# DUBSON0/iterative-closest-point-avmi

Hardware: AMD Instinct MI355X
Metric: icp_iterations_per_sec (higher is better)
Workload: dtype f64

## Files before the change

iterative-closest-point-avmi_amd/csrc/icp2.hip:

```cpp
#include <cstdlib>

#include "linalg.hpp"
#include "prep_common.hpp"
#include "sweep.hpp"

namespace icpmi {


struct Icp2Args {
    const double* pts;
    const int32_t* off;
    const int32_t* cnt;
    const int32_t* pair_src;
    const int32_t* pair_tgt;
    const double* init;
    double* results;
    const double2* g_sxy;
    const double2* g_snrm;
    const int32_t* g_sorig;
    const float* g_skey;
    const int32_t* g_dir;
    int lds_points;
    double error_threshold;
    double max_corr_dist;
    int max_iterations;
    int method;
    int has_init;
    int n_lo, m_lo;
    int skip_over;
    int it_begin, it_limit;
    int resume;
    double2* st_xy;
    int32_t* st_pos;
    int32_t* list;
    int32_t* list_count;
    int st_stride;
    int32_t* wide_list;
    int32_t* wide_count;
    int32_t* far_list;
    int32_t* far_count;
    double far_d2;
    IcpGate gate;
};
constexpr int ICP2_FAR_THREADS = 1024, ICP2_FAR_SMAX = 2, ICP2_FAR_POINTS = 2048;
constexpr int ICP2_ST_PARKED = 100;

__device__ __forceinline__ double swap_add(double a, double b, bool rows16) {
    const long long ab = __double_as_longlong(a), bb = __double_as_longlong(b);
    const unsigned alo = (unsigned)ab, ahi = (unsigned)(ab >> 32), blo = (unsigned)bb, bhi = (unsigned)(bb >> 32);
    unsigned xl, xh, yl, yh;
    if (rows16) {
        const auto r0 = __builtin_amdgcn_permlane16_swap(alo, blo, false, false);
        const auto r1 = __builtin_amdgcn_permlane16_swap(ahi, bhi, false, false);
        xl = r0[0]; yl = r0[1]; xh = r1[0]; yh = r1[1];
    } else {
        const auto r0 = __builtin_amdgcn_permlane32_swap(alo, blo, false, false);
        const auto r1 = __builtin_amdgcn_permlane32_swap(ahi, bhi, false, false);
        xl = r0[0]; yl = r0[1]; xh = r1[0]; yh = r1[1];
    }
    return __longlong_as_double(((long long)xh << 32) | xl) + __longlong_as_double(((long long)yh << 32) | yl);
}

constexpr int RED_MAXW = 16;
template <int NV>
constexpr int red_doubles() { return (NV + 3) / 4 * 4 * RED_MAXW; }

template <int NV>
__device__ __forceinline__ void wave_totals(double* scratch, const double (&v)[NV]) {
    constexpr int NP = (NV + 3) / 4 * 4;
    const int w = wave_id(), l = lane_id();
    double h[NP / 2];
#pragma unroll
    for (int j = 0; j < NP / 2; ++j)
        h[j] = swap_add(2 * j < NV ? v[2 * j] : 0.0, 2 * j + 1 < NV ? v[2 * j + 1] : 0.0, false);
#pragma unroll
    for (int k = 0; k < NP / 4; ++k) {
        const double q = row_sum(swap_add(h[2 * k], h[2 * k + 1], true));
        const int row = l >> 4;
        const int idx = 4 * k + ((row & 1) << 1) + (row >> 1);
        if ((l & 15) == 0 && idx < NV) scratch[idx * RED_MAXW + w] = q;
    }
}

template <int NV>
// ... 68 lines not shown
    ctrl[CTRL_TT] = (tt0 * r[0] + tt1 * r[1]) + t[0]; ctrl[CTRL_TT + 1] = (tt0 * r[2] + tt1 * r[3]) + t[1];
}

union FarSlot {
    struct { double x, y; int seed, pad; } in;
    struct { double s1, s3; int p1, p2; } out;
};
static_assert(sizeof(FarSlot) == 24, "24 B per row");

template <int THREADS, int ICP2_SMAX, bool TGT_LDS, bool FILT, bool RESUME, bool FAR = false>
__device__ __forceinline__ void icp2_pair(const Icp2Args& a, const int b) {
    extern __shared__ __attribute__((aligned(16))) unsigned char dyn[];
    __shared__ double redA[red_doubles<11>()];
    __shared__ double redB[red_doubles<4>()];
    __shared__ double ctrl[CTRL_DOUBLES];
    constexpr int NWAVES = THREADS / ICPMI_WAVE;

    const int tid = threadIdx.x;
    const bool lead = tid < ICPMI_WAVE;
    const int sc = a.pair_src[b], tc = a.pair_tgt[b];
    const int N = a.cnt ? a.cnt[sc] : a.off[sc + 1] - a.off[sc];
    const int M = a.cnt ? a.cnt[tc] : a.off[tc + 1] - a.off[tc];
    const double* src = a.pts + (size_t)a.off[sc] * 2;
    double* res = a.results + (size_t)b * ICPMI_RES_DOUBLES;
    const int dir = a.g_dir[tc];
    if (a.skip_over ? (N > THREADS * ICP2_SMAX || (TGT_LDS && M > a.lds_points)) : (a.n_lo >= 0 && N <= a.n_lo && M <= a.m_lo)) {
        if (a.skip_over && a.wide_list && threadIdx.x == 0) a.wide_list[atomicAdd(a.wide_count, 1)] = b;
        return;
    }
    const int gate_index = a.gate.base + b * a.gate.stride;
    if (RESUME && a.gate.hint) {
        __shared__ int gate_skip;
        if (tid == 0) {
            gate_skip = __hip_atomic_load(a.gate.hint, __ATOMIC_RELAXED, __HIP_MEMORY_SCOPE_AGENT) < gate_index;
            if (gate_skip) {
                res[ICPMI_RES_ITERS] += 1.0;
                res[ICPMI_RES_STATUS] = (double)ICPMI_ST_SKIPPED;
            }
        }
        __syncthreads();
        if (gate_skip) return;
    }

    double2* lds_xy = reinterpret_cast<double2*>(dyn);
    double2* lds_nrm = reinterpret_cast<double2*>(dyn + (size_t)a.lds_points * 16);
    int32_t* lds_orig = reinterpret_cast<int32_t*>(dyn + (size_t)a.lds_points * 32);
    float4* lds_sq = reinterpret_cast<float4*>(dyn + (size_t)a.lds_points * 32) + 1;
    const double2* sxy = TGT_LDS ? lds_xy : a.g_sxy + a.off[tc];
    const double2* snrm = TGT_LDS ? lds_nrm : a.g_snrm + a.off[tc];
    const int32_t* sorig = TGT_LDS ? lds_orig : a.g_sorig + a.off[tc];
    static_assert(TGT_LDS || !FILT, "the filter images live in LDS");
    static_assert(!FAR || (FILT && RESUME), "the far continuation: filter images, parked state");
    float4* lds_tree = reinterpret_cast<float4*>(dyn + (size_t)a.lds_points * 48 + 32);
    const int tree_leaves = sweepf_tree_leaves(M);
    FarSlot* far_q = reinterpret_cast<FarSlot*>(dyn + (size_t)a.lds_points * 50 + 32) + (size_t)(threadIdx.x / ICPMI_WAVE) * (ICPMI_WAVE * ICP2_SMAX);
    __shared__ int rt_bits;
    if (FILT && tid == 0) rt_bits = 0;

    if (tid == 0) {
        if (RESUME) {
            ctrl[CTRL_RT] = res[0]; ctrl[CTRL_RT + 1] = res[1]; ctrl[CTRL_RT + 2] = res[2]; ctrl[CTRL_RT + 3] = res[3];
            ctrl[CTRL_TT] = res[ICPMI_RES_T]; ctrl[CTRL_TT + 1] = res[ICPMI_RES_T + 1];
            ctrl[CTRL_ERR] = res[ICPMI_RES_ERR]; ctrl[CTRL_PREV] = res[ICPMI_RES_ERR]; ctrl[CTRL_DELTA] = res[ICPMI_RES_DELTA];
            ctrl[CTRL_ITERS] = res[ICPMI_RES_ITERS];
        } else {
            const double* in = a.init + (size_t)b * 6;
            ctrl[CTRL_RT] = a.has_init ? in[0] : 1.0; ctrl[CTRL_RT + 1] = a.has_init ? in[1] : 0.0;
            ctrl[CTRL_RT + 2] = a.has_init ? in[2] : 0.0; ctrl[CTRL_RT + 3] = a.has_init ? in[3] : 1.0;
            ctrl[CTRL_TT] = a.has_init ? in[4] : 0.0; ctrl[CTRL_TT + 1] = a.has_init ? in[5] : 0.0;
            ctrl[CTRL_ERR] = __builtin_inf(); ctrl[CTRL_PREV] = __builtin_inf(); ctrl[CTRL_DELTA] = __builtin_inf();
            ctrl[CTRL_ITERS] = 0.0;
        }
        ctrl[CTRL_STATUS] = (double)ICPMI_ST_MAXITER;
    }

    if (N <= 0 || M <= 0 || dir < 0 || (TGT_LDS && M > a.lds_points) || N > THREADS * ICP2_SMAX || (!FILT && dir >= SWEEP_POLAR)) {
        if (tid == 0) ctrl[CTRL_STATUS] = (double)ICPMI_ST_EMPTY;
    } else {
        const bool use_p2l = a.method == ICPMI_POINT_TO_LINE;
        const double2* gx = a.g_sxy + a.off[tc];
        const double2* gn = a.g_snrm + a.off[tc];
        const int32_t* go = a.g_sorig + a.off[tc];
        const float* gk = a.g_skey + a.off[tc];
        SweepF filt{0.0, 0.0, 0.0, 0.0f, 0.0f};
        if constexpr (TGT_LDS && !FILT)
            for (int i = tid; i < M; i += THREADS) {
                lds_xy[i] = gx[i];
                lds_orig[i] = go[i];
                if (use_p2l) lds_nrm[i] = gn[i];
            }
        if constexpr (FILT) {
            if (dir != SWEEP_POLAR) {
                const double2 o = gx[M >> 1];
                filt.ox = wave_uniform(o.x); filt.oy = wave_uniform(o.y); filt.uo = wave_uniform(proj(dir, o.x, o.y));
            }
            float rmax = 0.0f;
            for (int i = tid; i < M; i += THREADS) {
                const double2 p = gx[i];
                lds_xy[i] = p;
                if (use_p2l) lds_nrm[i] = gn[i];
                const float4 q = make_float4((float)(p.x - filt.ox), (float)(p.y - filt.oy),
                                             dir == SWEEP_POLAR ? gk[i] : (float)(proj(dir, p.x, p.y) - filt.uo),
                                             __int_as_float(go[i]));
                lds_sq[i] = q;
                rmax = fmaxf(rmax, fmaxf(fabsf(q.x), fabsf(q.y)));
            }
            if (tid == 0) { lds_sq[-1] = make_float4(0.f, 0.f, 0.f, 0.f); lds_sq[M] = make_float4(0.f, 0.f, 0.f, 0.f); }
            __syncthreads();
            atomicMax(&rt_bits, __float_as_int(rmax));
        }
        double px[ICP2_SMAX], py[ICP2_SMAX];
        int pos[ICP2_SMAX];
        float ax[ICP2_SMAX], ay[ICP2_SMAX], budget[ICP2_SMAX];
        int pos2[ICP2_SMAX];
#pragma unroll
        for (int s = 0; s < ICP2_SMAX; ++s) { ax[s] = 0.0f; ay[s] = 0.0f; budget[s] = -1.0f; pos2[s] = -1; }
        const int S = (N + THREADS - 1) / THREADS;
#pragma unroll
        for (int s = 0; s < ICP2_SMAX; ++s) {
            const int n = s * THREADS + tid;
            px[s] = 0.0; py[s] = 0.0; pos[s] = -1;
            if (n < N && RESUME) {
                const double2 v = a.st_xy[(size_t)b * a.st_stride + n];
                px[s] = v.x; py[s] = v.y; pos[s] = a.st_pos[(size_t)b * a.st_stride + n];
            } else if (n < N) {
                const double x = src[2 * n], y = src[2 * n + 1];
                if (a.has_init) {
                    const double* in = a.init + (size_t)b * 6;
                    double sx = 0.0, sy = 0.0;
                    sx += x * in[0]; sx += y * in[1]; sx += in[4];
                    sy += x * in[2]; sy += y * in[3]; sy += in[5];
                    px[s] = sx; py[s] = sy;
                } else { px[s] = x; py[s] = y; }
            }
        }
        const bool has_corr = a.max_corr_dist >= 0.0;
        const double max_corr_sq = wave_uniform(a.max_corr_dist * a.max_corr_dist);
        const int need = max(3, N / 10);
        __syncthreads();
        if constexpr (FAR) {
            sweepf_build_tree(lds_sq, M, lds_tree, tree_leaves, tid, THREADS);
            __syncthreads();
        }
        const double2 c_lo = sxy[0], c_hi = sxy[M - 1];
        const double uabs = wave_uniform(fmax(fabs(proj(dir, c_lo.x, c_lo.y)), fabs(proj(dir, c_hi.x, c_hi.y))));
        if constexpr (FILT) {
            filt.rt = wave_uniform(__int_as_float(rt_bits) * 1.000001f);
            filt.ut = wave_uniform(fmaxf(fabsf(lds_sq[0].z), fabsf(lds_sq[M - 1].z)) * 1.000001f);
        }

        double e_part = 0.0;
        if (RESUME) {
#pragma unroll
            for (int s = 0; s < ICP2_SMAX; ++s) {
                if (!(s < S && s * THREADS + tid < N)) continue;
                const double2 q = sxy[pos[s]];
                const double ex = q.x - px[s], ey = q.y - py[s];
                double se = 0.0;
                se += ex * ex;
                se += ey * ey;
                e_part += se;
            }
// ... 58 lines not shown
                                pos[s] = sweepf_nn_pk(lds_sq, sxy, filt, M, dir, uabs, px[s], py[s], pos[s], it < ICP2_PLAIN_CENTRED);
                            else pos[s] = sweepf_nn(lds_sq, sxy, filt, M, dir, uabs, px[s], py[s], pos[s], it < ICP2_PLAIN_CENTRED, d2s);
                        }
                        else pos[s] = sweep_nn(sxy, sorig, M, dir, uabs, px[s], py[s], pos[s], it < ICP2_PLAIN_CENTRED, d2s);
                    }
            } else {
                const bool centred = !RESUME && it < ICP2_CENTRED_ITERS;
                int slot[ICP2_SMAX];
                if constexpr (FAR) {
                    int nq = 0;
#pragma unroll
                    for (int s = 0; s < ICP2_SMAX; ++s) {
                        const unsigned long long bal = __ballot(srch[s]);
                        slot[s] = nq + (int)__builtin_amdgcn_mbcnt_hi((unsigned)(bal >> 32), __builtin_amdgcn_mbcnt_lo((unsigned)bal, 0u));
                        nq += __popcll(bal);
                        if (srch[s]) {
                            FarSlot e;
                            e.in.x = px[s]; e.in.y = py[s]; e.in.seed = pos[s]; e.in.pad = 0;
                            far_q[slot[s]] = e;
                        }
                    }
                    __builtin_amdgcn_fence(__ATOMIC_ACQ_REL, "wavefront");
                    __builtin_amdgcn_wave_barrier();
                    for (int j = tid & (ICPMI_WAVE - 1); j < nq; j += ICPMI_WAVE) {
                        const FarSlot e = far_q[j];
                        const Top2 r = sweepf_top2_far(lds_sq, sxy, lds_tree, tree_leaves, filt, M, dir, uabs, e.in.x, e.in.y, e.in.seed);
                        FarSlot o;
                        o.out.s1 = r.s1; o.out.s3 = r.s3; o.out.p1 = r.p1; o.out.p2 = r.p2;
                        far_q[j] = o;
                    }
                    __builtin_amdgcn_fence(__ATOMIC_ACQ_REL, "wavefront");
                    __builtin_amdgcn_wave_barrier();
                }
#pragma unroll
                for (int s = 0; s < ICP2_SMAX; ++s)
                    if (srch[s]) {
                        Top2 t2;
                        if constexpr (FAR) {
                            const FarSlot o = far_q[slot[s]];
                            t2.p1 = o.out.p1; t2.p2 = o.out.p2; t2.s1 = o.out.s1; t2.s2 = o.out.s1; t2.s3 = o.out.s3;
                        }
                        else if constexpr (FILT) {
                            if (__popcll(__ballot(true)) >= ICP2_PK_MIN)
                                t2 = sweepf_top2_pk(lds_sq, sxy, filt, M, dir, uabs, px[s], py[s], pos[s], centred);
                            else t2 = sweepf_top2(lds_sq, sxy, filt, M, dir, uabs, px[s], py[s], pos[s], centred);
                        }
                        else t2 = sweep_top2(sxy, sorig, M, dir, uabs, px[s], py[s], pos[s], centred);
                        pos[s] = t2.p1; pos2[s] = t2.p2;
                        float bf;
                        if constexpr (FAR) {
                            const double d1 = sqrt(t2.s1), d3 = sqrt(t2.s3);
                            bf = (float)(d3 - 1e-13 * (d3 + d1) - 1.3e-7 * (fabs(px[s]) + fabs(py[s])));
                        } else {
                            const float r3 = __builtin_amdgcn_sqrtf((float)t2.s3) * 0.9999997f;
                            const float r1 = __builtin_amdgcn_sqrtf((float)t2.s1) * 1.0000003f + 1e-30f;
                            bf = (r3 - r1) * 0.4999999f - 1.3e-7f * (fabsf((float)px[s]) + fabsf((float)py[s]));
                        }
                        bf = bf - fabsf(bf) * 1e-6f;
                        budget[s] = t2.s3 < __builtin_inf() ? bf : __builtin_inff();
                        ax[s] = (float)px[s]; ay[s] = (float)py[s];
                    }
            }
            bool in[ICP2_SMAX];
#pragma unroll
            for (int s = 0; s < ICP2_SMAX; ++s) in[s] = s < S && s * THREADS + tid < N;
            if (use_p2l) {
                double acc[11] = {0, 0, 0, 0, 0, 0, 0, 0, 0, 0, 0};
#pragma unroll
                for (int s = 0; s < ICP2_SMAX; ++s) {
                    if (!in[s]) continue;
                    const double2 q = sxy[pos[s]], nm = snrm[pos[s]];
                    const double dx = px[s] - q.x, dy = py[s] - q.y;
                    if (has_corr) {
                        double s2 = 0.0;
                        s2 += dx * dx;
                        s2 += dy * dy;
                        const double dist = sqrt(s2);
                        if (!(dist * dist < max_corr_sq)) continue;
                    }
                    const double c = nm.y * px[s] - nm.x * py[s];
                    const double bi = -(nm.x * dx + nm.y * dy);
                    acc[0] += c * c;       acc[1] += c * nm.x;    acc[2] += c * nm.y;
                    acc[3] += nm.x * nm.x; acc[4] += nm.x * nm.y; acc[5] += nm.y * nm.y;
                    acc[6] += c * bi;      acc[7] += nm.x * bi;   acc[8] += nm.y * bi;
                    acc[9] += 1.0;
                }
                acc[10] = e_part;
                wave_totals<11>(redA, acc);
                __syncthreads();
                if (lead) {
                    combine_totals<11>(redA, NWAVES, acc);
                    const int fin = gate_stop(ctrl, a.gate.hint, gate_seen, gate_index, tid == 0,
                                              finish_step(ctrl, it, acc[10], acc[9], N, has_corr, need, a.error_threshold, tid == 0, far_err));
                    const bool stop = fin == FIN_STOP;
                    if (!stop) {
                        double A[3][3] = {{acc[0], acc[1], acc[2]}, {acc[1], acc[3], acc[4]}, {acc[2], acc[4], acc[5]}};
                        double rhs[3] = {acc[6], acc[7], acc[8]}, x[3];
                        double r[4], t[2];
                        if (solve3(A, rhs, x)) {
                            double st, ct;
                            sincos_step(x[0], st, ct);
                            r[0] = ct; r[1] = -st; r[2] = st; r[3] = ct; t[0] = x[1]; t[1] = x[2];
                        } else {
                            r[0] = 1.0; r[1] = 0.0; r[2] = 0.0; r[3] = 1.0; t[0] = 0.0; t[1] = 0.0;
                        }
                        if (tid == 0) {
                            accumulate_step(ctrl, r, t);
                            ctrl[CTRL_R] = r[0]; ctrl[CTRL_R + 1] = r[1]; ctrl[CTRL_R + 2] = r[2]; ctrl[CTRL_R + 3] = r[3];
                            ctrl[CTRL_T] = t[0]; ctrl[CTRL_T + 1] = t[1];
// ... 156 lines not shown
    for (int j = first + blockIdx.x; j < count; j += gridDim.x) {
        icp2_pair<THREADS, ICP2_SMAX, TGT_LDS, FILT, true>(a, __builtin_amdgcn_readfirstlane(a.list[j]));
        __syncthreads();
    }
}

__global__ __launch_bounds__(ICP2_FAR_THREADS, 4) void icp2_far_kernel(Icp2Args a) {
    const int count = *a.far_count;
    for (int j = blockIdx.x; j < count; j += gridDim.x) {
        icp2_pair<ICP2_FAR_THREADS, ICP2_FAR_SMAX, true, true, true, true>(a, __builtin_amdgcn_readfirstlane(a.far_list[j]));
        __syncthreads();
    }
}

struct Icp2Ws {
    Carve c;
    int n_pairs, max_src_n;
    size_t st_rows = (size_t)n_pairs * (size_t)max_src_n;
    double2* st_xy = c.packed<double2>(st_rows * 16);
    int32_t* st_pos = c.packed<int32_t>(st_rows * 4);
    int32_t *list = c.packed<int32_t>((size_t)n_pairs * 4), *wide_list = c.packed<int32_t>((size_t)n_pairs * 4);
    int32_t* far_list = c.packed<int32_t>((size_t)n_pairs * 4);
    int32_t* list_count = c.packed<int32_t>(64);
    size_t bytes = c.off;
};


struct Icp2Shape {
    int threads, smax;
    bool in_lds, filter;
    int lds_points;
    size_t lds;
    int n_lo, m_lo;
    int skip_over;
};
struct Icp2Plan {
    Icp2Shape first;
    bool has_wide;
    Icp2Shape wide;
    bool two_stage;
    int stage1_iterations, stage2_grid, wide_grid;
    bool far_wanted;
    Icp2Shape far;
    double far_d2;
    bool needs_lists;
};
constexpr int ICP2_NO_LIMIT = 0x7fffffff;

static Icp2Shape icp2_shape(int threads, int smax, int points, bool in_lds) {
    int cap = 64;
    while (cap < points) cap <<= 1;
    if (points > 1024 && points <= 1536) cap = 1536;
    const bool filter = in_lds && cap <= 2048;
    const size_t lds = in_lds ? (filter ? (size_t)cap * 48 + 32 : (size_t)cap * 36) : 0;
    return {threads, smax, in_lds, filter, cap, lds, -1, 0, 0};
}

static Icp2Plan plan_icp2(int n_pairs, int max_src_n, int max_tgt_n, const icpmi_icp_params& p, bool have_ws,
                          const char* stages_opt, const char* far_opt) {
    Icp2Plan plan{};
    const bool in_lds = max_tgt_n <= 4096;
    const bool many = n_pairs >= 1024;
    int T, SM;
    if (max_src_n <= 1024) { T = 512; SM = 2; }
    else if (many) { T = 768; SM = 2; }
    else if (max_src_n <= 2048) { T = 1024; SM = 2; }
    else { T = 1024; SM = 4; }
    const int cap1 = ((T == 512 || T == 768) && many && in_lds && max_tgt_n > 1536) ? 1536 : max_tgt_n;
    plan.first = icp2_shape(T, SM, cap1, in_lds);
    plan.has_wide = T * SM < max_src_n || cap1 < max_tgt_n;
    if (plan.has_wide) {
        plan.first.skip_over = 1;
        plan.wide = icp2_shape(1024, max_src_n <= 2048 ? 2 : 4, max_tgt_n, in_lds);
        plan.wide.n_lo = T * SM; plan.wide.m_lo = cap1;
    }
    plan.stage1_iterations = ICP2_STAGE1_ITERS;
    plan.two_stage = many && have_ws && p.max_iterations >= 2 * plan.stage1_iterations &&
                     !(stages_opt && stages_opt[0] == '1') &&
                     (p.method == ICPMI_POINT_TO_LINE || (stages_opt && stages_opt[0] == '2'));
    plan.stage2_grid = n_pairs / 8 > 256 ? n_pairs / 8 : 256;
    plan.wide_grid = n_pairs < 256 ? n_pairs : (n_pairs / 32 > 256 ? n_pairs / 32 : 256);
    plan.far_d2 = far_opt ? atof(far_opt) : 1.0;
    plan.far_wanted = have_ws && in_lds && plan.far_d2 > 0.0 && p.max_iterations > 2;
    int far_cap = 64;
    while (far_cap < max_tgt_n && far_cap < ICP2_FAR_POINTS) far_cap <<= 1;
    plan.far = {ICP2_FAR_THREADS, ICP2_FAR_SMAX, true, true, far_cap,
                (size_t)far_cap * 50 + 32 + sizeof(FarSlot) * (size_t)(ICP2_FAR_THREADS * ICP2_FAR_SMAX), -1, 0, 0};
    plan.needs_lists = have_ws && (plan.two_stage || plan.has_wide);
    return plan;
}

struct Icp2Kernels {
    void (*fused)(Icp2Args);
    void (*wide)(Icp2Args);
    void (*resume)(Icp2Args);
    void (*resume_rest)(Icp2Args, int);
};
template <int T, int S, bool L, bool F>
constexpr Icp2Kernels icp2_kernels() {
    return {icp2_fused_kernel<T, S, L, F>, icp2_wide_kernel<T, S, L, F>, icp2_resume_kernel<T, S, L, F>,
            icp2_resume_rest_kernel<T, S, L, F>};
}
template <int T, int S>
static Icp2Kernels icp2_kernels_of(const Icp2Shape& s) {
    if (!s.in_lds) return icp2_kernels<T, S, false, false>();
    if (s.filter) return icp2_kernels<T, S, true, true>();
    return icp2_kernels<T, S, true, false>();
}
static Icp2Kernels icp2_kernels_of(const Icp2Shape& s) {
    if (s.threads == 512 && s.smax == 2) return icp2_kernels_of<512, 2>(s);
    if (s.threads == 768 && s.smax == 2) return icp2_kernels_of<768, 2>(s);
    if (s.threads == 1024 && s.smax == 2) return icp2_kernels_of<1024, 2>(s);
    if (s.threads == 1024 && s.smax == 4) return icp2_kernels_of<1024, 4>(s);
    return {nullptr, nullptr, nullptr, nullptr};
}

static Icp2Args icp2_args(const Icp2Args& base, const Icp2Shape& s, int it_begin, int it_limit, int resume) {
    Icp2Args a = base;
    a.lds_points = s.lds_points; a.n_lo = s.n_lo; a.m_lo = s.m_lo; a.skip_over = s.skip_over;
    a.it_begin = it_begin; a.it_limit = it_limit; a.resume = resume;
    return a;
}

int launch_icp2(const double* pts, const int32_t* off, const int32_t* cnt, const int32_t* ps, const int32_t* pt,
                int n_pairs, int max_src_n, int max_tgt_n, int total_rows, const icpmi_icp_params* p, const double* init,
                double* results, const void* prepared, void* workspace, size_t workspace_bytes, const IcpGate* gate,
                hipStream_t st) {
    const Icp2Ws w{workspace, n_pairs, max_src_n};
    const bool have_ws = workspace && workspace_bytes >= w.bytes;
    const Icp2Plan plan = plan_icp2(n_pairs, max_src_n, max_tgt_n, *p, have_ws, option("ICP2_STAGES"), option("ICP2_FAR"));
    const Icp2Kernels k1 = icp2_kernels_of(plan.first), k2 = icp2_kernels_of(plan.wide);
    if (!k1.fused || (plan.has_wide && !k2.fused)) return ICPMI_ERR_ARG;
    Icp2Args base;
    base.gate = gate ? *gate : IcpGate{nullptr, nullptr, 0.0, 0, 1};
    base.st_xy = nullptr; base.st_pos = nullptr; base.list = nullptr; base.list_count = nullptr; base.st_stride = 0;
    base.wide_list = nullptr; base.wide_count = nullptr;
    base.far_list = nullptr; base.far_count = nullptr; base.far_d2 = __builtin_inf();
    const PreparedView v(prepared, total_rows);
    base.pts = pts; base.off = off; base.cnt = cnt; base.pair_src = ps; base.pair_tgt = pt; base.init = init; base.results = results;
    base.g_sxy = v.sxy; base.g_snrm = v.snrm; base.g_sorig = v.sorig; base.g_skey = v.skey; base.g_dir = v.dir;
    base.error_threshold = p->error_threshold; base.max_corr_dist = p->max_corr_dist;
    base.max_iterations = p->max_iterations; base.method = p->method; base.has_init = p->has_init;
    const bool far_go = plan.far_wanted && dyn_lds((const void*)icp2_far_kernel, plan.far.lds) == hipSuccess;
    if (plan.needs_lists || far_go) {
        base.st_xy = w.st_xy; base.st_pos = w.st_pos; base.st_stride = max_src_n;
        base.list = w.list; base.list_count = w.list_count;
        if (plan.has_wide) { base.wide_list = w.wide_list; base.wide_count = w.list_count + 1; }
        if (far_go) { base.far_list = w.far_list; base.far_count = w.list_count + 2; base.far_d2 = plan.far_d2; }
        if (hipMemsetAsync(w.list_count, 0, 3 * sizeof(int32_t), st) != hipSuccess) return ICPMI_ERR_HIP;
    }
    SideLock side_lock;
    Side* const side = side_lock.side;

    const Icp2Shape& s1 = plan.first;
    if (dyn_lds((const void*)k1.fused, s1.lds) != hipSuccess) return ICPMI_ERR_HIP;
    k1.fused<<<n_pairs, s1.threads, s1.lds, st>>>(
        icp2_args(base, s1, 0, plan.two_stage ? plan.stage1_iterations : ICP2_NO_LIMIT, 0));
    bool forked = false;
    if (plan.two_stage) {
        if (base.wide_list && side) forked = hipEventRecord(side->fork, st) == hipSuccess;
        const Icp2Args second = icp2_args(base, s1, plan.stage1_iterations, ICP2_NO_LIMIT, 1);
        if (dyn_lds((const void*)k1.resume, s1.lds) != hipSuccess) return ICPMI_ERR_HIP;
        k1.resume<<<plan.stage2_grid, s1.threads, s1.lds, st>>>(second);
        if (plan.stage2_grid < n_pairs) {
            if (dyn_lds((const void*)k1.resume_rest, s1.lds) != hipSuccess) return ICPMI_ERR_HIP;
            k1.resume_rest<<<256, s1.threads, s1.lds, st>>>(second, plan.stage2_grid);
        }
    }
    if (plan.has_wide) {
        const Icp2Shape& s2 = plan.wide;
        const Icp2Args wide = icp2_args(base, s2, 0, ICP2_NO_LIMIT, 0);
        if (base.wide_list) {
            if (dyn_lds((const void*)k2.wide, s2.lds) != hipSuccess) return ICPMI_ERR_HIP;
            hipStream_t ws = st;
            if (forked && hipStreamWaitEvent(side->stream[0], side->fork, 0) == hipSuccess) ws = side->stream[0];
            k2.wide<<<plan.wide_grid, s2.threads, s2.lds, ws>>>(wide);
            if (ws != st && (hipEventRecord(side->join[0], ws) != hipSuccess ||
                             hipStreamWaitEvent(st, side->join[0], 0) != hipSuccess)) {
                (void)hipStreamSynchronize(ws);
                return ICPMI_ERR_HIP;
            }
        } else {
            if (dyn_lds((const void*)k2.fused, s2.lds) != hipSuccess) return ICPMI_ERR_HIP;
            k2.fused<<<n_pairs, s2.threads, s2.lds, st>>>(wide);
        }
    }
    if (base.far_list)
// ... 8 lines not shown
```

iterative-closest-point-avmi_amd/csrc/prep.hip:

```cpp
#include "prep_common.hpp"

namespace icpmi {

#ifndef PREP_AXIS_STEP
#define PREP_AXIS_STEP 4
#endif
#ifndef ICPMI_PREP_WPS
#define ICPMI_PREP_WPS 6
#endif
constexpr int PREP_THREADS = 512;
constexpr int PREP_MAXW = PREP_THREADS / ICPMI_WAVE;
constexpr int PREP_MAX_POINTS = 4096;

constexpr float PREP_POLAR_Q = 6.283185307179586f / 2097152.0f;
__device__ __forceinline__ uint32_t prep_polar_key21(double x, double y) {
    const float t = (atan2f((float)y, (float)x) + 3.14159265f) * (2097152.0f / 6.283185307179586f);
    const int k = (int)t;
    return (uint32_t)(k < 0 ? 0 : (k > 2097151 ? 2097151 : k));
}
__device__ __forceinline__ float prep_polar_image(uint32_t k21) { return (float)k21 * PREP_POLAR_Q - 3.14159265f; }

template <int E>
__device__ __forceinline__ void prep_sort_polar32(const double* __restrict__ P, int M, uint64_t* keys, uint32_t* rows) {
    uint32_t v[E];
#pragma unroll
    for (int e = 0; e < E; ++e) {
        const int i = e * PREP_THREADS + (int)threadIdx.x;
        v[e] = i < M ? (prep_polar_key21(P[2 * i], P[2 * i + 1]) << 11) | (uint32_t)i : 0xffffffffu;
    }
    bitonic_sort_regs_fixed<uint32_t, E, PREP_THREADS>(v, reinterpret_cast<uint32_t*>(keys));
    __syncthreads();
#pragma unroll
    for (int e = 0; e < E; ++e) {
        const int i = (int)threadIdx.x * E + e;
        rows[i] = v[e] == 0xffffffffu ? 0xffffffffu : (v[e] & 0x7ffu);
        keys[i] = v[e] == 0xffffffffu ? ~0ull : f64_sortable((double)prep_polar_image(v[e] >> 11));
    }
    __syncthreads();
}

template <int E>
__device__ __forceinline__ void prep_sort_regs(const double* __restrict__ P, int M, int dir, uint64_t* by_row, uint64_t* keys,
                                               uint32_t* rows) {
    if (dir == SWEEP_POLAR) { prep_sort_polar32<E>(P, M, keys, rows); return; }
    constexpr uint64_t ROW_MASK = 0x7ff;
    uint64_t v[E];
#pragma unroll
    for (int e = 0; e < E; ++e) {
        const int i = (int)threadIdx.x * E + e;
        const uint64_t k = i < M ? f64_sortable(proj(dir, P[2 * i], P[2 * i + 1])) : ~0ull;
        by_row[i] = k;
        v[e] = i < M ? ((k & ~ROW_MASK) | (uint64_t)i) : ~0ull;
    }
    bitonic_sort_regs_fixed<uint64_t, E, PREP_THREADS>(v, keys);
    int bad = 0;
#pragma unroll
    for (int e = 0; e < E; ++e) {
        const int i = (int)threadIdx.x * E + e;
        const uint32_t r = v[e] == ~0ull ? 0xffffffffu : (uint32_t)(v[e] & ROW_MASK);
        rows[i] = r;
        keys[i] = r == 0xffffffffu ? ~0ull : by_row[r];
    }
    __syncthreads();
#pragma unroll
    for (int e = 0; e < E; ++e) {
        const int i = (int)threadIdx.x * E + e;
        if (i + 1 < M && (keys[i] > keys[i + 1] || (keys[i] == keys[i + 1] && rows[i] > rows[i + 1]))) bad = 1;
    }
    if (__syncthreads_or(bad)) {
        if (threadIdx.x == 0)
            for (int i = 1; i < M; ++i) {
                const uint64_t k = keys[i];
                const uint32_t r = rows[i];
                int j = i - 1;
                while (j >= 0 && (keys[j] > k || (keys[j] == k && rows[j] > r))) { keys[j + 1] = keys[j]; rows[j + 1] = rows[j]; --j; }
                keys[j + 1] = k; rows[j + 1] = r;
            }
        __syncthreads();
    }
}

template <int KK, bool GRID>
__global__ __launch_bounds__(PREP_THREADS, (KK <= 13 ? ICPMI_PREP_WPS : (KK <= 16 ? 4 : 2))) void prep_targets_kernel(
    const double* __restrict__ pts, const int32_t* __restrict__ off, const int32_t* __restrict__ cnt,
    const int32_t* __restrict__ cloud_ids, int k, double2* __restrict__ g_sxy, double2* __restrict__ g_snrm,
    int32_t* __restrict__ g_sorig, float* __restrict__ g_skey, int32_t* __restrict__ g_dir, double* __restrict__ out_normals,
    int lds_points, int split, int polar) {
    extern __shared__ __attribute__((aligned(16))) unsigned char dyn[];
    __shared__ double dsc[8 * PREP_MAXW];
// ... 276 lines not shown
```

iterative-closest-point-avmi_amd/csrc/state.hip:

```cpp
#include <link.h>

#include <cstdio>
#include <cstdlib>
#include <cstring>
#include <map>
#include <set>
#include <mutex>
#include <string>

#include "common.hpp"

namespace icpmi {

static const char* const kOptionNames[] = {"ICP2_SIDE", "ICP2_FAR", "ICP2_STAGES", "POLAR", "PREP_KNN", "RAYCAST", "RS_BATCH"};

struct Options {
    std::mutex mu;
    bool loaded = false;
    std::map<std::string, std::string> values;
    void load() {
        if (loaded) return;
        loaded = true;
        for (const char* n : kOptionNames) {
            const std::string env = std::string("ICPMI_") + n;
            if (const char* v = getenv(env.c_str())) values[n] = v;
        }
    }
};
static Options& options() { static Options o; return o; }

static const char* strip_prefix(const char* name) { return strncmp(name, "ICPMI_", 6) == 0 ? name + 6 : name; }

const char* option(const char* name) {
    Options& o = options();
    std::lock_guard<std::mutex> g(o.mu);
    o.load();
    const auto it = o.values.find(strip_prefix(name));
    return it == o.values.end() ? nullptr : it->second.c_str();
}

struct LdsAttr {
    std::mutex mu;
    std::map<std::pair<const void*, int>, size_t> granted;
};
static LdsAttr& lds_attr() { static LdsAttr a; return a; }

hipError_t dyn_lds(const void* fn, size_t bytes) {
    int dev = -1;
    hipError_t e = hipGetDevice(&dev);
    if (e != hipSuccess) return e;
    LdsAttr& a = lds_attr();
    std::lock_guard<std::mutex> g(a.mu);
    size_t& have = a.granted[std::make_pair(fn, dev)];
    if (bytes <= have) return hipSuccess;
    e = hipFuncSetAttribute(fn, hipFuncAttributeMaxDynamicSharedMemorySize, (int)bytes);
    if (e == hipSuccess) have = bytes;
    return e;
}

struct SideState {
    std::mutex mu;
    std::map<int, Side> per_device;
};
static SideState& side_state() { static SideState s; return s; }

SideLock::SideLock() : side(nullptr) {
    SideState& s = side_state();
// ... 74 lines not shown
```

iterative-closest-point-avmi_amd/csrc/sweep.hpp:

```cpp
#pragma once
#include "common.hpp"

namespace icpmi {

__device__ __forceinline__ double proj(int dir, double x, double y) {
    const double a = dir == 1 ? 0.0 : 1.0;
    const double b = dir == 0 ? 0.0 : (dir == 3 ? -1.0 : 1.0);
    return x * a + y * b;
}

__device__ __forceinline__ bool gap_exceeds(int dir, double uq, double uc, double bound_d2) {
    const double du = fabs(uq - uc);
    if (dir < 2) return du * du > bound_d2;
    const double e = 4.5e-16 * (fabs(uq) + fabs(uc));
    const double l = du - e;
    return l > 0.0 && l * l > bound_d2 * 2.000000000000002;
}

__device__ __forceinline__ int sweep_lower_bound(const double2* sxy, int m, int dir, double uq) {
    int lo = 0, hi = m;
    while (lo < hi) {
        const int mid = (lo + hi) >> 1;
        const double2 c = sxy[mid];
        if (proj(dir, c.x, c.y) < uq) lo = mid + 1; else hi = mid;
// ... 136 lines not shown
        lo = inl ? lo - 1 : -1;
        cr = nr; cl = nl;
    }
    return t;
}

__device__ __forceinline__ int sweep_nn(const double2* sxy, const int32_t* sorig, int m, int dir, double uabs,
                                        double qx, double qy, int seed, bool CENTRED, double& d2_out) {
    const SweepAxis ax(dir, qx, qy, uabs);
    double best = __builtin_inf(), thr = __builtin_inf();
    int bpos = 0;
    int lo, hi;
    const bool seeded = seed >= 0 && seed < m;
    if (seeded) {
        best = sweep_d2(qx, qy, sxy[seed]); bpos = seed;
        thr = ax.width(best);
    }
    if (seeded && !CENTRED) { lo = seed - 1; hi = seed + 1; }
    else {
        hi = sweep_lower_bound(sxy, m, dir, ax.uq);
        lo = hi - 1;
    }
    double2 cr = sweep_load(sxy, hi, m), cl = sweep_load(sxy, lo, m);
    while (lo >= 0 || hi < m) {
        const double2 nr = sweep_load(sxy, hi + 1, m), nl = sweep_load(sxy, lo - 1, m);
        const bool inr = hi < m && !(ax.u(cr) - ax.uq > thr);
        const bool inl = lo >= 0 && !(ax.uq - ax.u(cl) > thr);
        const double sr = sweep_d2(qx, qy, cr), sl = sweep_d2(qx, qy, cl);
#pragma unroll
        for (int side = 0; side < 2; ++side) {
            const int i = side == 0 ? hi : lo;
            const double s = side == 0 ? sr : sl;
            const bool take = side == 0 ? inr : inl;
            if (take && s == best && i != bpos) {
                if (sorig[i] < sorig[bpos]) bpos = i;
            }
            const bool lt = take && s < best;
            best = lt ? s : best;
            bpos = lt ? i : bpos;
        }
        thr = ax.width(best);
        hi = inr ? hi + 1 : m;
        lo = inl ? lo - 1 : -1;
        cr = nr; cl = nl;
    }
    d2_out = best;
    return bpos;
}


constexpr int SWEEP_POLAR = 4;
__device__ __forceinline__ double polar_key(double x, double y) { return atan2(y, x); }

struct SweepF {
    double ox, oy, uo;
    float ut, rt;
};
struct SweepFQuery {
    float x, y, u;
    float e15, mu;
    float kw;
    bool polar;
    __device__ __forceinline__ SweepFQuery(const SweepF& f, int dir, double uabs, double qx, double qy) {
        polar = dir == SWEEP_POLAR;
        x = (float)(qx - f.ox); y = (float)(qy - f.oy);
        e15 = 1.8e-7f * (fabsf(x) + fabsf(y) + 2.0f * f.rt) + 1e-30f;
        if (polar) {
            u = atan2f(y, x);
            mu = 1e-5f;
            kw = 1.00001f / __builtin_amdgcn_sqrtf(x * x + y * y);
        } else {
            const SweepAxis ax(dir, qx, qy, uabs);
            u = (float)(ax.uq - f.uo);
            mu = 2.4e-7f * (fabsf(u) + f.ut) + (float)ax.slack * 1.000001f + 1e-30f;
            kw = dir < 2 ? 1.0f : 1.4142137f;
        }
    }
    __device__ __forceinline__ void bounds(double best, float& W, float& T) const {
        const float B = __builtin_amdgcn_sqrtf((float)best) * 1.000001f + 1e-18f;
        const float t = B * kw;
        if (polar) W = t <= 0.7f ? (t + 0.3f * t * t * t) * 1.000001f + mu : __builtin_inff();
        else W = t * 1.000001f + mu;
        const float b = B + e15;
        T = b * b * 1.000002f;
    }
};

typedef float sweep_v2f __attribute__((ext_vector_type(2)));

__device__ __forceinline__ int sweepf_row(const float4 c) { return __float_as_int(c.w); }

__device__ __forceinline__ int sweepf_lower_bound(const float4* sq, int m, float u) {
    int lo = 0, hi = m;
    while (lo < hi) {
        const int mid = (lo + hi) >> 1;
        if (sq[mid].z < u) lo = mid + 1; else hi = mid;
    }
    return lo;
}

struct SweepFWalk {
    int lo, hi, lo_end, hi_end;
    bool openr, openl;
    sweep_v2f uu;
    __device__ __forceinline__ SweepFWalk(int lo0, int hi0, int m, float u) {
        lo = lo0; hi = hi0; lo_end = -1; hi_end = m; openr = true; openl = true;
        uu = sweep_v2f{-u, u};
    }
    __device__ __forceinline__ bool more() const { return (openr && hi < hi_end) || (openl && lo > lo_end); }
    __device__ __forceinline__ bool wrap(int m) {
        const bool endr = openr && hi >= hi_end, endl = openl && lo <= lo_end;
        if (endr == endl) return false;
        if (endr) { hi_end = lo + 1; hi = 0; uu.x += 6.2831855f; openl = false; lo_end = lo; }
        else { lo_end = hi - 1; lo = m - 1; uu.y += 6.2831855f; openr = false; hi_end = hi; }
        return hi < hi_end || lo > lo_end;
    }
};

struct SweepFRound {
    bool inr, inl, pr, pl;
    float4 cr, cl;
    __device__ __forceinline__ SweepFRound(const float4* sq, const SweepFWalk& w, const SweepFQuery& fq, float W, float T) {
        cr = sq[w.hi]; cl = sq[w.lo];
        const sweep_v2f cz = {cr.z, -cl.z};
        const sweep_v2f g = cz + w.uu;
        inr = w.openr && w.hi < w.hi_end && !(g.x > W);
        inl = w.openl && w.lo > w.lo_end && !(g.y > W);
        const sweep_v2f cx = {cr.x, cl.x}, cy = {cr.y, cl.y};
        const sweep_v2f dx = fq.x - cx, dy = fq.y - cy;
        const sweep_v2f s2 = __builtin_elementwise_fma(dx, dx, dy * dy);
        pr = inr && !(s2.x > T);
        pl = inl && !(s2.y > T);
    }
    __device__ __forceinline__ void advance(SweepFWalk& w) const {
        w.openr = w.openr && (inr || w.hi >= w.hi_end);
        w.openl = w.openl && (inl || w.lo <= w.lo_end);
        w.hi += inr ? 1 : 0;
        w.lo -= inl ? 1 : 0;
    }
};

__device__ __forceinline__ int sweepf_nn(const float4* sq, const double2* sxy, const SweepF& f, int m, int dir, double uabs,
                                         double qx, double qy, int seed, bool CENTRED, double& d2_out) {
    const SweepFQuery fq(f, dir, uabs, qx, qy);
    double best = __builtin_inf();
    float W = __builtin_inff(), T = __builtin_inff();
    int bpos = 0;
    const bool seeded = seed >= 0 && seed < m;
    if (seeded) {
        best = sweep_d2(qx, qy, sxy[seed]); bpos = seed;
        fq.bounds(best, W, T);
    }
    const bool from_seed = seeded && !CENTRED && !(fq.polar && fabsf(sq[seed].z - fq.u) > 3.0f);
    const int h0 = from_seed ? seed + 1 : sweepf_lower_bound(sq, m, fq.u);
    SweepFWalk w(from_seed ? seed - 1 : h0 - 1, h0, m, fq.u);
#pragma unroll 1
    for (int pass = 0; pass < 2; ++pass) {
        while (w.more()) {
            const SweepFRound r(sq, w, fq, W, T);
            if (r.pr || r.pl) {
#pragma unroll
                for (int side = 0; side < 2; ++side) {
                    const int i = side == 0 ? w.hi : w.lo;
                    if (side == 0 ? r.pr : r.pl) {
                        const double s = sweep_d2(qx, qy, sxy[i]);
                        if (s == best && i != bpos) {
                            if (sweepf_row(side == 0 ? r.cr : r.cl) < sweepf_row(sq[bpos])) bpos = i;
                        }
                        if (s < best) { best = s; bpos = i; }
                    }
                }
                fq.bounds(best, W, T);
            }
            r.advance(w);
        }
        if (!fq.polar || !w.wrap(m)) break;
    }
    d2_out = best;
    return bpos;
}

__device__ __forceinline__ Top2 sweepf_top2(const float4* sq, const double2* sxy, const SweepF& f, int m, int dir, double uabs,
                                            double qx, double qy, int seed, bool CENTRED) {
    const SweepFQuery fq(f, dir, uabs, qx, qy);
    Top2 t;
    t.p1 = 0; t.p2 = -1;
    t.s1 = t.s2 = t.s3 = __builtin_inf();
    float W = __builtin_inff(), T = __builtin_inff();
    const bool seeded = seed >= 0 && seed < m;
    if (seeded) { t.s1 = sweep_d2(qx, qy, sxy[seed]); t.p1 = seed; }
    const bool from_seed = seeded && !CENTRED && !(fq.polar && fabsf(sq[seed].z - fq.u) > 3.0f);
    const int h0 = from_seed ? seed + 1 : sweepf_lower_bound(sq, m, fq.u);
    SweepFWalk w(from_seed ? seed - 1 : h0 - 1, h0, m, fq.u);
    const int skip = seeded ? seed : -1;
#pragma unroll 1
    for (int pass = 0; pass < 2; ++pass) {
        while (w.more()) {
            const SweepFRound r(sq, w, fq, W, T);
            const bool pr = r.pr && w.hi != skip, pl = r.pl && w.lo != skip;
            if (pr || pl) {
#pragma unroll
                for (int side = 0; side < 2; ++side) {
                    const int i = side == 0 ? w.hi : w.lo;
                    if (side == 0 ? pr : pl) {
                        const double s = sweep_d2(qx, qy, sxy[i]);
                        if (s == t.s1 || s == t.s2) {
                            const int row = sweepf_row(side == 0 ? r.cr : r.cl), r1 = sweepf_row(sq[t.p1]);
                            const int r2 = t.p2 >= 0 ? sweepf_row(sq[t.p2]) : 0x7fffffff;
                            if (s < t.s1 || (s == t.s1 && row < r1)) { t.s3 = t.s2; t.s2 = t.s1; t.p2 = t.p1; t.s1 = s; t.p1 = i; }
                            else if (s < t.s2 || row < r2) { t.s3 = t.s2; t.s2 = s; t.p2 = i; }
                            else t.s3 = s;
                        } else {
                            const bool c1 = s < t.s1, c2 = s < t.s2, c3 = s < t.s3;
                            t.s3 = c2 ? t.s2 : (c3 ? s : t.s3);
                            t.s2 = c1 ? t.s1 : (c2 ? s : t.s2);
                            t.p2 = c1 ? t.p1 : (c2 ? i : t.p2);
                            t.s1 = c1 ? s : t.s1;
                            t.p1 = c1 ? i : t.p1;
                        }
                    }
                }
                fq.bounds(t.s3, W, T);
            }
            r.advance(w);
        }
        if (!fq.polar || !w.wrap(m)) break;
    }
    return t;
}

constexpr unsigned SWEEP_PK_IDX = 0x7FFu;
constexpr unsigned SWEEP_PK_NONE = 0xFFFFFFFFu;

__device__ __forceinline__ unsigned sweep_med3_u32(unsigned a, unsigned b, unsigned c) {
    unsigned r;
    asm("v_med3_u32 %0, %1, %2, %3" : "=v"(r) : "v"(a), "v"(b), "v"(c));
    return r;
}
__device__ __forceinline__ unsigned sweep_min_u32(unsigned a, unsigned b) { return a < b ? a : b; }

template <int K>
struct SweepPkList {
    unsigned m[K];
    __device__ __forceinline__ SweepPkList() {
#pragma unroll
// ... 24 lines not shown
    __device__ __forceinline__ float width(float B) const {
        const float t = B * kw;
        if (POLAR) {
            const float w = __builtin_fmaf(t, __builtin_fmaf(0.3000004f, t * t, 1.000001f), mu);
            return t <= 0.7f ? w : __builtin_inff();
        }
        return __builtin_fmaf(t, 1.000001f, mu);
    }
    __device__ __forceinline__ float threshold(float B) const {
        const float b = B + e15;
        return b * b * 1.000002f;
    }
};

template <int K, int NB, bool POLAR>
__device__ __forceinline__ bool sweep_pk_walk(const float4* sq, const SweepPkQuery& fq, int lo, int hi, int m, int skip, SweepPkList<K>& L,
                                              int max_rounds = 0) {
    float W = fq.width<POLAR>(fq.dist_bound(L.m[NB]));
    const float ur = -fq.u, ul = fq.u, ur2 = 6.2831855f - fq.u, ul2 = fq.u + 6.2831855f;
    int rounds = 0;
    for (;;) {
        int hp = hi, lp = lo;
        float o_r = ur, o_l = ul;
        bool okr, okl;
        if (POLAR) {
            const bool wr = hi >= m, wl = lo < 0;
            hp = wr ? hi - m : hi;
            lp = wl ? lo + m : lo;
            o_r = wr ? ur2 : ur;
            o_l = wl ? ul2 : ul;
            okr = hi - lo <= m;
        } else {
            okr = hi < m;
            okl = lo >= 0;
        }
        const float4 cr = sq[hp], cl = sq[lp];
        const bool inr = okr && !(cr.z + o_r > W);
        if (POLAR) okl = hi + (inr ? 1 : 0) - lo <= m;
        const bool inl = okl && !(o_l - cl.z > W);
        const sweep_v2f cx = {cr.x, cl.x}, cy = {cr.y, cl.y};
        const sweep_v2f dx = fq.x - cx, dy = fq.y - cy;
        const sweep_v2f s2 = __builtin_elementwise_fma(dx, dx, dy * dy);
        L.offer(sweep_pk(s2.x, hp, inr && hp != skip));
        L.offer(sweep_pk(s2.y, lp, inl && lp != skip));
        if (!(inr || inl)) return true;
        if (max_rounds > 0 && ++rounds >= max_rounds) return false;
        W = fq.width<POLAR>(fq.dist_bound(L.m[NB]));
        hi += inr ? 1 : 0;
        lo -= inl ? 1 : 0;
    }
}

template <int K, int NB>
__device__ __forceinline__ void sweep_pk_search(const float4* sq, const SweepPkQuery& fq, int m, int seed, bool CENTRED, SweepPkList<K>& L) {
    const bool seeded = seed >= 0 && seed < m;
    int skip = -1;
    const bool from_seed = seeded && !CENTRED && !(fq.polar && fabsf(sq[seed].z - fq.u) > 3.0f);
    if (seeded && !from_seed) {
        const float4 c = sq[seed];
        const float ex = fq.x - c.x, ey = fq.y - c.y;
        L.offer(sweep_pk(__builtin_fmaf(ex, ex, ey * ey), seed, true));
        skip = seed;
    }
    const int h0 = from_seed ? seed + 1 : sweepf_lower_bound(sq, m, fq.u);
    if (fq.polar) sweep_pk_walk<K, NB, true>(sq, fq, h0 - 1, h0, m, skip, L);
    else sweep_pk_walk<K, NB, false>(sq, fq, h0 - 1, h0, m, skip, L);
}

__device__ __forceinline__ int sweepf_nn_pk(const float4* sq, const double2* sxy, const SweepF& f, int m, int dir, double uabs,
                                            double qx, double qy, int seed, bool CENTRED) {
    const SweepPkQuery fq(f, dir, uabs, qx, qy);
    SweepPkList<3> L;
    sweep_pk_search<3, 0>(sq, fq, m, seed, CENTRED, L);
    const float T = fq.threshold(fq.dist_bound(L.m[0]));
    int bpos = (int)(L.m[0] & SWEEP_PK_IDX);
    const bool a2 = L.m[1] != SWEEP_PK_NONE && !(sweep_pk_floor(L.m[1]) > T);
    const bool a3 = L.m[2] != SWEEP_PK_NONE && !(sweep_pk_floor(L.m[2]) > T);
    if (a3 || fq.bad || L.m[0] == SWEEP_PK_NONE) {
        double d2;
        bpos = sweepf_nn(sq, sxy, f, m, dir, uabs, qx, qy, seed, CENTRED, d2);
    } else if (a2) {
        const int i2 = (int)(L.m[1] & SWEEP_PK_IDX);
        const double s1 = sweep_d2(qx, qy, sxy[bpos]), s2 = sweep_d2(qx, qy, sxy[i2]);
        if (s2 < s1 || (s2 == s1 && sweepf_row(sq[i2]) < sweepf_row(sq[bpos]))) bpos = i2;
    }
    return bpos;
}

__device__ __forceinline__ Top2 sweep_pk_top2_exact(const float4* sq, const double2* sxy, double qx, double qy, unsigned w0, unsigned w1, unsigned w2) {
    const unsigned w[3] = {w0, w1, w2};
    double s[3];
    int p[3], r[3];
#pragma unroll
    for (int k = 0; k < 3; ++k) {
        const bool have = w[k] != SWEEP_PK_NONE;
        p[k] = have ? (int)(w[k] & SWEEP_PK_IDX) : -1;
        const int j = have ? p[k] : 0;
        s[k] = have ? sweep_d2(qx, qy, sxy[j]) : __builtin_inf();
        r[k] = have ? sweepf_row(sq[j]) : 0x7fffffff;
    }
#define ICPMI_CS(a, b)                                                                              \
    do {                                                                                            \
        const bool sw = s[b] < s[a] || (s[b] == s[a] && r[b] < r[a]);                              \
        const double sa = sw ? s[b] : s[a], sb = sw ? s[a] : s[b];                                  \
        const int pa = sw ? p[b] : p[a], pb = sw ? p[a] : p[b], ra = sw ? r[b] : r[a], rb = sw ? r[a] : r[b]; \
        s[a] = sa; s[b] = sb; p[a] = pa; p[b] = pb; r[a] = ra; r[b] = rb;                           \
    } while (0)
    ICPMI_CS(0, 1); ICPMI_CS(1, 2); ICPMI_CS(0, 1);
#undef ICPMI_CS
    Top2 t;
    t.p1 = p[0]; t.p2 = p[1]; t.s1 = s[0]; t.s2 = s[1]; t.s3 = s[2];
    return t;
}

__device__ __forceinline__ Top2 sweepf_top2_pk(const float4* sq, const double2* sxy, const SweepF& f, int m, int dir, double uabs,
                                               double qx, double qy, int seed, bool CENTRED) {
    const SweepPkQuery fq(f, dir, uabs, qx, qy);
    SweepPkList<4> L;
    sweep_pk_search<4, 2>(sq, fq, m, seed, CENTRED, L);
    const float T = fq.threshold(fq.dist_bound(L.m[2]));
    const bool a4 = L.m[3] != SWEEP_PK_NONE && !(sweep_pk_floor(L.m[3]) > T);
    if (a4 || fq.bad || L.m[0] == SWEEP_PK_NONE) return sweepf_top2(sq, sxy, f, m, dir, uabs, qx, qy, seed, CENTRED);
    return sweep_pk_top2_exact(sq, sxy, qx, qy, L.m[0], L.m[1], L.m[2]);
}

constexpr int SWEEP_BLOCK = 16;
#ifndef SWEEP_FAR_ROUNDS
#define SWEEP_FAR_ROUNDS 24
#endif

__host__ __device__ __forceinline__ int sweepf_tree_leaves(int m) {
    int l = 2;
    while (l * SWEEP_BLOCK < m) l <<= 1;
    return l;
}

__device__ __forceinline__ void sweepf_build_tree(const float4* sq, int m, float4* tree, int leaves, int tid, int nthreads) {
    for (int b = tid; b < leaves; b += nthreads) {
        const int i1 = min(m, (b + 1) * SWEEP_BLOCK);
        float x0 = __builtin_inff(), y0 = __builtin_inff(), x1 = -__builtin_inff(), y1 = -__builtin_inff();
        for (int i = b * SWEEP_BLOCK; i < i1; ++i) {
            const float4 c = sq[i];
            x0 = fminf(x0, c.x); y0 = fminf(y0, c.y); x1 = fmaxf(x1, c.x); y1 = fmaxf(y1, c.y);
        }
        tree[leaves + b] = make_float4(x0, y0, x1, y1);
    }
    __syncthreads();
    for (int k = 1 + tid; k < leaves; k += nthreads) {
        int lo = k, hi = k;
        while (lo < leaves) { lo = 2 * lo; hi = 2 * hi + 1; }
        float x0 = __builtin_inff(), y0 = __builtin_inff(), x1 = -__builtin_inff(), y1 = -__builtin_inff();
        for (int j = lo; j <= hi; ++j) {
            const float4 c = tree[j];
            x0 = fminf(x0, c.x); y0 = fminf(y0, c.y); x1 = fmaxf(x1, c.z); y1 = fmaxf(y1, c.w);
        }
        tree[k] = make_float4(x0, y0, x1, y1);
    }
}

__device__ __forceinline__ float sweepf_box_s2(const float4 bb, float qx, float qy) {
    const float dx = fmaxf(fmaxf(bb.x - qx, qx - bb.z), 0.0f), dy = fmaxf(fmaxf(bb.y - qy, qy - bb.w), 0.0f);
    return __builtin_fmaf(dx, dx, dy * dy);
}

template <class Offer>
__device__ __forceinline__ void sweepf_far_scan(const float4* sq, const float4* tree, int leaves, int m, const SweepFQuery& fq,
                                                const float& T, Offer offer) {
    int node = 1;
    unsigned trail = 0;
    bool tested = true;
    for (;;) {
        bool down = tested || !(sweepf_box_s2(tree[node], fq.x, fq.y) > T);
// ... 226 lines not shown
```

Baseline: 42.00 million.

## Add LDS bucket table to accelerate sweep lower-bound searches

Builds a 2048-entry uint16 bucket index over the sorted sweep keys in LDS, so the lower-bound binary search only scans inside one bucket instead of the whole target array. It is enabled by default for non-resume filter launches and can be switched off with an ICP2_BUCKETS option. It adds LDS footprint and a build pass per block, which may reduce occupancy and, for seeded queries that skip the lower bound, may cost more than it saves. The change also bundles a double-precision fallback for budget computation when distances are huge, and a fix in prep that marks padding rows by index rather than by sentinel value.

```diff
diff --git a/iterative-closest-point-avmi_amd/csrc/icp2.hip b/iterative-closest-point-avmi_amd/csrc/icp2.hip
--- a/iterative-closest-point-avmi_amd/csrc/icp2.hip
+++ b/iterative-closest-point-avmi_amd/csrc/icp2.hip
@@ -30,6 +30,7 @@
     int skip_over;
     int it_begin, it_limit;
     int resume;
+    int buckets;
     double2* st_xy;
     int32_t* st_pos;
     int32_t* list;
@@ -204,6 +205,7 @@
     static_assert(TGT_LDS || !FILT, "the filter images live in LDS");
     static_assert(!FAR || (FILT && RESUME), "the far continuation: filter images, parked state");
     float4* lds_tree = reinterpret_cast<float4*>(dyn + (size_t)a.lds_points * 48 + 32);
+    uint16_t* lds_bucket = reinterpret_cast<uint16_t*>(dyn + (size_t)a.lds_points * 48 + 32);
     const int tree_leaves = sweepf_tree_leaves(M);
     FarSlot* far_q = reinterpret_cast<FarSlot*>(dyn + (size_t)a.lds_points * 50 + 32) + (size_t)(threadIdx.x / ICPMI_WAVE) * (ICPMI_WAVE * ICP2_SMAX);
     __shared__ int rt_bits;
@@ -260,6 +262,11 @@
             if (tid == 0) { lds_sq[-1] = make_float4(0.f, 0.f, 0.f, 0.f); lds_sq[M] = make_float4(0.f, 0.f, 0.f, 0.f); }
             __syncthreads();
             atomicMax(&rt_bits, __float_as_int(rmax));
+            if constexpr (!RESUME)
+                if (a.buckets) {
+                    const SweepBuckets bk = sweepf_build_buckets(lds_sq, M, lds_bucket, tid, THREADS);
+                    filt.bk.tab = bk.tab; filt.bk.lo = wave_uniform(bk.lo); filt.bk.scale = wave_uniform(bk.scale);
+                }
         }
         double px[ICP2_SMAX], py[ICP2_SMAX];
         int pos[ICP2_SMAX];
@@ -424,9 +431,14 @@
                             const double d1 = sqrt(t2.s1), d3 = sqrt(t2.s3);
                             bf = (float)(d3 - 1e-13 * (d3 + d1) - 1.3e-7 * (fabs(px[s]) + fabs(py[s])));
                         } else {
-                            const float r3 = __builtin_amdgcn_sqrtf((float)t2.s3) * 0.9999997f;
-                            const float r1 = __builtin_amdgcn_sqrtf((float)t2.s1) * 1.0000003f + 1e-30f;
-                            bf = (r3 - r1) * 0.4999999f - 1.3e-7f * (fabsf((float)px[s]) + fabsf((float)py[s]));
+                            if (t2.s3 < 1e30) {
+                                const float r3 = __builtin_amdgcn_sqrtf((float)t2.s3) * 0.9999997f;
+                                const float r1 = __builtin_amdgcn_sqrtf((float)t2.s1) * 1.0000003f + 1e-18f;
+                                bf = (r3 - r1) * 0.4999999f - 1.3e-7f * (fabsf((float)px[s]) + fabsf((float)py[s]));
+                            } else {
+                                const double d1 = sqrt(t2.s1), d3 = sqrt(t2.s3);
+                                bf = (float)((d3 - d1) * 0.4999999995 - 1e-13 * (d3 + d1) - 1.3e-7 * (fabs(px[s]) + fabs(py[s])));
+                            }
                         }
                         bf = bf - fabsf(bf) * 1e-6f;
                         budget[s] = t2.s3 < __builtin_inf() ? bf : __builtin_inff();
@@ -689,7 +701,7 @@
     while (cap < points) cap <<= 1;
     if (points > 1024 && points <= 1536) cap = 1536;
     const bool filter = in_lds && cap <= 2048;
-    const size_t lds = in_lds ? (filter ? (size_t)cap * 48 + 32 : (size_t)cap * 36) : 0;
+    const size_t lds = in_lds ? (filter ? (size_t)cap * 48 + 32 + SWEEP_BUCKET_BYTES : (size_t)cap * 36) : 0;
     return {threads, smax, in_lds, filter, cap, lds, -1, 0, 0};
 }
 
@@ -756,6 +768,7 @@
     Icp2Args a = base;
     a.lds_points = s.lds_points; a.n_lo = s.n_lo; a.m_lo = s.m_lo; a.skip_over = s.skip_over;
     a.it_begin = it_begin; a.it_limit = it_limit; a.resume = resume;
+    a.buckets = base.buckets && s.filter && !resume;
     return a;
 }
 
@@ -770,6 +783,8 @@
     if (!k1.fused || (plan.has_wide && !k2.fused)) return ICPMI_ERR_ARG;
     Icp2Args base;
     base.gate = gate ? *gate : IcpGate{nullptr, nullptr, 0.0, 0, 1};
+    const char* buckets_opt = option("ICP2_BUCKETS");
+    base.buckets = !(buckets_opt && buckets_opt[0] == '0');
     base.st_xy = nullptr; base.st_pos = nullptr; base.list = nullptr; base.list_count = nullptr; base.st_stride = 0;
     base.wide_list = nullptr; base.wide_count = nullptr;
     base.far_list = nullptr; base.far_count = nullptr; base.far_d2 = __builtin_inf();
diff --git a/iterative-closest-point-avmi_amd/csrc/prep.hip b/iterative-closest-point-avmi_amd/csrc/prep.hip
--- a/iterative-closest-point-avmi_amd/csrc/prep.hip
+++ b/iterative-closest-point-avmi_amd/csrc/prep.hip
@@ -33,8 +33,9 @@
 #pragma unroll
     for (int e = 0; e < E; ++e) {
         const int i = (int)threadIdx.x * E + e;
-        rows[i] = v[e] == 0xffffffffu ? 0xffffffffu : (v[e] & 0x7ffu);
-        keys[i] = v[e] == 0xffffffffu ? ~0ull : f64_sortable((double)prep_polar_image(v[e] >> 11));
+        const bool pad = i >= M;
+        rows[i] = pad ? 0xffffffffu : (v[e] & 0x7ffu);
+        keys[i] = pad ? ~0ull : f64_sortable((double)prep_polar_image(v[e] >> 11));
     }
     __syncthreads();
 }
diff --git a/iterative-closest-point-avmi_amd/csrc/state.hip b/iterative-closest-point-avmi_amd/csrc/state.hip
--- a/iterative-closest-point-avmi_amd/csrc/state.hip
+++ b/iterative-closest-point-avmi_amd/csrc/state.hip
@@ -12,7 +12,7 @@
 
 namespace icpmi {
 
-static const char* const kOptionNames[] = {"ICP2_SIDE", "ICP2_FAR", "ICP2_STAGES", "POLAR", "PREP_KNN", "RAYCAST", "RS_BATCH"};
+static const char* const kOptionNames[] = {"ICP2_BUCKETS", "ICP2_SIDE", "ICP2_FAR", "ICP2_STAGES", "POLAR", "PREP_KNN", "RAYCAST", "RS_BATCH"};
 
 struct Options {
     std::mutex mu;
diff --git a/iterative-closest-point-avmi_amd/csrc/sweep.hpp b/iterative-closest-point-avmi_amd/csrc/sweep.hpp
--- a/iterative-closest-point-avmi_amd/csrc/sweep.hpp
+++ b/iterative-closest-point-avmi_amd/csrc/sweep.hpp
@@ -212,9 +212,20 @@
 constexpr int SWEEP_POLAR = 4;
 __device__ __forceinline__ double polar_key(double x, double y) { return atan2(y, x); }
 
+constexpr int SWEEP_BUCKETS = 2048;
+constexpr size_t SWEEP_BUCKET_BYTES = ((size_t)(SWEEP_BUCKETS + 1) * 2 + 15) / 16 * 16;
+struct SweepBuckets {
+    const uint16_t* tab = nullptr;
+    float lo = 0.0f, scale = 0.0f;
+    __device__ __forceinline__ int bin(float key) const {
+        return (int)fminf(fmaxf((key - lo) * scale, 0.0f), (float)(SWEEP_BUCKETS - 1));
+    }
+};
+
 struct SweepF {
     double ox, oy, uo;
     float ut, rt;
+    SweepBuckets bk;
 };
 struct SweepFQuery {
     float x, y, u;
@@ -259,6 +270,33 @@
     return lo;
 }
 
+__device__ __forceinline__ int sweepf_lower_bound(const float4* sq, int m, float u, const SweepBuckets& bk) {
+    if (!bk.tab) return sweepf_lower_bound(sq, m, u);
+    const int b = bk.bin(u);
+    int lo = bk.tab[b], hi = bk.tab[b + 1];
+    while (lo < hi) {
+        const int mid = (lo + hi) >> 1;
+        if (sq[mid].z < u) lo = mid + 1; else hi = mid;
+    }
+    return lo;
+}
+
+__device__ __forceinline__ SweepBuckets sweepf_build_buckets(const float4* sq, int m, uint16_t* tab, int tid, int nthreads) {
+    SweepBuckets bk;
+    bk.tab = tab;
+    bk.lo = sq[0].z;
+    const float range = sq[m - 1].z - bk.lo;
+    bk.scale = range > 0.0f ? (float)SWEEP_BUCKETS / range : 0.0f;
+    if (!(bk.scale < 3.0e38f)) bk.scale = 0.0f;
+    for (int i = tid; i < m; i += nthreads) {
+        const int b1 = bk.bin(sq[i].z);
+        for (int b = i > 0 ? bk.bin(sq[i - 1].z) + 1 : 0; b <= b1; ++b) tab[b] = (uint16_t)i;
+        if (i == m - 1)
+            for (int b = b1 + 1; b <= SWEEP_BUCKETS; ++b) tab[b] = (uint16_t)m;
+    }
+    return bk;
+}
+
 struct SweepFWalk {
     int lo, hi, lo_end, hi_end;
     bool openr, openl;
@@ -312,7 +350,7 @@
         fq.bounds(best, W, T);
     }
     const bool from_seed = seeded && !CENTRED && !(fq.polar && fabsf(sq[seed].z - fq.u) > 3.0f);
-    const int h0 = from_seed ? seed + 1 : sweepf_lower_bound(sq, m, fq.u);
+    const int h0 = from_seed ? seed + 1 : sweepf_lower_bound(sq, m, fq.u, f.bk);
     SweepFWalk w(from_seed ? seed - 1 : h0 - 1, h0, m, fq.u);
 #pragma unroll 1
     for (int pass = 0; pass < 2; ++pass) {
@@ -350,7 +388,7 @@
     const bool seeded = seed >= 0 && seed < m;
     if (seeded) { t.s1 = sweep_d2(qx, qy, sxy[seed]); t.p1 = seed; }
     const bool from_seed = seeded && !CENTRED && !(fq.polar && fabsf(sq[seed].z - fq.u) > 3.0f);
-    const int h0 = from_seed ? seed + 1 : sweepf_lower_bound(sq, m, fq.u);
+    const int h0 = from_seed ? seed + 1 : sweepf_lower_bound(sq, m, fq.u, f.bk);
     SweepFWalk w(from_seed ? seed - 1 : h0 - 1, h0, m, fq.u);
     const int skip = seeded ? seed : -1;
 #pragma unroll 1
@@ -481,7 +519,8 @@
 }
 
 template <int K, int NB>
-__device__ __forceinline__ void sweep_pk_search(const float4* sq, const SweepPkQuery& fq, int m, int seed, bool CENTRED, SweepPkList<K>& L) {
+__device__ __forceinline__ void sweep_pk_search(const float4* sq, const SweepPkQuery& fq, const SweepBuckets& bk, int m, int seed, bool CENTRED,
+                                                SweepPkList<K>& L) {
     const bool seeded = seed >= 0 && seed < m;
     int skip = -1;
     const bool from_seed = seeded && !CENTRED && !(fq.polar && fabsf(sq[seed].z - fq.u) > 3.0f);
@@ -491,7 +530,7 @@
         L.offer(sweep_pk(__builtin_fmaf(ex, ex, ey * ey), seed, true));
         skip = seed;
     }
-    const int h0 = from_seed ? seed + 1 : sweepf_lower_bound(sq, m, fq.u);
+    const int h0 = from_seed ? seed + 1 : sweepf_lower_bound(sq, m, fq.u, bk);
     if (fq.polar) sweep_pk_walk<K, NB, true>(sq, fq, h0 - 1, h0, m, skip, L);
     else sweep_pk_walk<K, NB, false>(sq, fq, h0 - 1, h0, m, skip, L);
 }
@@ -500,7 +539,7 @@
                                             double qx, double qy, int seed, bool CENTRED) {
     const SweepPkQuery fq(f, dir, uabs, qx, qy);
     SweepPkList<3> L;
-    sweep_pk_search<3, 0>(sq, fq, m, seed, CENTRED, L);
+    sweep_pk_search<3, 0>(sq, fq, f.bk, m, seed, CENTRED, L);
     const float T = fq.threshold(fq.dist_bound(L.m[0]));
     int bpos = (int)(L.m[0] & SWEEP_PK_IDX);
     const bool a2 = L.m[1] != SWEEP_PK_NONE && !(sweep_pk_floor(L.m[1]) > T);
@@ -546,7 +585,7 @@
                                                double qx, double qy, int seed, bool CENTRED) {
     const SweepPkQuery fq(f, dir, uabs, qx, qy);
     SweepPkList<4> L;
-    sweep_pk_search<4, 2>(sq, fq, m, seed, CENTRED, L);
+    sweep_pk_search<4, 2>(sq, fq, f.bk, m, seed, CENTRED, L);
     const float T = fq.threshold(fq.dist_bound(L.m[2]));
     const bool a4 = L.m[3] != SWEEP_PK_NONE && !(sweep_pk_floor(L.m[3]) > T);
     if (a4 || fq.bad || L.m[0] == SWEEP_PK_NONE) return sweepf_top2(sq, sxy, f, m, dir, uabs, qx, qy, seed, CENTRED);
```

After: 42.20 million (median of 6 runs). About the same (+0.5%).
